# CatchMan1/AI-education-generative-recommendation

Measured on AMD Instinct MI355X. Metric: RQ-VAE items encoded/s + SASRec seqs scored/s @1/8 GPU; HR@10/NDCG@10 parity, higher is better.
Workload: dtype f32; 1 GPU; rq_c2: RQ-VAE get_indices, 3x256 codebooks, in 768 -> [256,128] -> e 32, data-derived codebooks, BERT-statistics item embeddings; global_batch=100000, parallelism=item-sharded x1, no collective

## Files before the change

ai-education-generative-recommendation_amd/_lib.py:

```python
import ctypes
import os

import torch

_PKG = os.path.dirname(os.path.abspath(__file__))
LIB_PATH = os.environ.get("GR_AMD_LIB") or os.path.join(_PKG, "lib", "libgr_amd.so")

GR_ACT_NONE = 0
GR_ACT_RELU = 1
GR_ACT_SIGMOID = 2
GR_ACT_TANH = 3
GR_ACT_LEAKYRELU = 4
GR_MAX_LEVELS = 8
GR_MAX_LINEAR = 8

_c_int_p = ctypes.POINTER(ctypes.c_int32)
_vp = ctypes.c_void_p
_i64 = ctypes.c_int64
_i32 = ctypes.c_int32
_sz = ctypes.c_size_t
_f32 = ctypes.c_float


class SasrecParams(ctypes.Structure):
    _fields_ = [("d", _i32), ("n_blocks", _i32), ("n_heads", _i32), ("mlp", _i32),
                ("max_len", _i32), ("eps", _f32), ("item_rows", _i64),
                ("item_emb", _vp), ("pos_emb", _vp),
                ("attn_ln_w", _vp), ("attn_ln_b", _vp), ("in_proj_w", _vp), ("in_proj_b", _vp),
                ("out_proj_w", _vp), ("out_proj_b", _vp), ("ffn_ln_w", _vp), ("ffn_ln_b", _vp),
                ("ffn1_w", _vp), ("ffn1_b", _vp), ("ffn2_w", _vp), ("ffn2_b", _vp),
                ("last_ln_w", _vp), ("last_ln_b", _vp)]


class SasrecTrainBufs(ctypes.Structure):
    _fields_ = [(f, _vp) for f in ("xin", "hs", "qkv", "prob", "os", "x1", "fs", "zs", "us", "xl", "g_vec")]


SIGNATURES = {
    "gr_version": (ctypes.c_char_p, []),
    "gr_last_error": (ctypes.c_char_p, []),
    "gr_set_option": (ctypes.c_int, [ctypes.c_char_p, _i64]),
    "gr_get_option": (_i64, [ctypes.c_char_p]),
    "gr_linear_f32": (ctypes.c_int, [_vp, _i64, _i32, _vp, _i32, _vp, _vp, _i64, _i32, _vp, _i64, _vp]),
    "gr_rq_codebook_norms_f32": (ctypes.c_int, [_vp, _i32, _i32, _vp, _vp]),
    "gr_rq_quantize_f32": (ctypes.c_int, [_vp, _i64, _i32, _i32, _vp, _vp, _vp, _vp, _vp, _vp, _vp]),
    "gr_rq_encode_workspace_bytes": (_sz, [_i64, _i32, _vp, _i32, _vp]),
    "gr_rq_encode_f32": (ctypes.c_int, [_vp, _i64, _i32, _vp, _vp, _vp, _i32, _vp, _vp, _vp, _vp,
                                        _vp, _vp, _vp, _sz, _vp]),
    "gr_rq_encoder_pack_floats": (_sz, [_i32, _vp]),
    "gr_rq_encoder_pack_f32": (ctypes.c_int, [_i32, _vp, _vp, _vp, _vp]),
    "gr_rq_encode_packed_f32": (ctypes.c_int, [_vp, _i64, _i32, _vp, _vp, _vp, _vp, _i32, _vp, _vp, _vp,
                                               _vp, _vp, _vp, _vp, _sz, _vp]),
    "gr_rq_mlp_workspace_bytes": (_sz, [_i64, _i32, _vp]),
    "gr_rq_mlp_f32": (ctypes.c_int, [_vp, _i64, _i32, _vp, _vp, _vp, _vp, _vp, _sz, _vp]),
    "gr_mlp_exact_f32": (ctypes.c_int, [_vp, _i64, _i32, _vp, _vp, _vp, _vp, _vp, _vp, _vp, _f32, _i32,
                                        _vp, _vp, _sz, _vp]),
    "gr_mlp_exact_groups_f32": (ctypes.c_int, [_vp, _i64, _i32, _vp, _vp, _vp, _vp, _vp, _vp, _vp, _f32,
                                               _i32, _vp, _i64, _vp, _vp]),
    "gr_mkl_plan": (_i32, [_i64, _i32, _i32, _c_int_p, _c_int_p]),
    "gr_rq_encode_sk_workspace_bytes": (_sz, [_i64, _i32, _i32, _vp]),
    "gr_rq_encode_sk_f32": (ctypes.c_int, [_vp, _i64, _i32, _i32, _vp, _vp, _vp, _i32, _vp, _i64,
                                           _vp, _vp, _sz, _vp]),
    "gr_mlp_train_fwd_f32": (ctypes.c_int, [_vp, _i64, _i32, _vp, _vp, _vp, _f32, _vp, _vp, _vp, _vp]),
    "gr_mlp_train_bwd_layer_f32": (ctypes.c_int, [_vp, _i64, _i32, _vp, _i32, _vp, _i32, _f32, _vp, _i32,
                                                  _vp, _vp, _vp, _vp]),
    "gr_rq_quantize_sk_train_f32": (ctypes.c_int, [_vp, _i64, _i32, _i32, _vp, _vp, _vp, _i32, _vp, _i64,
                                                   _vp, _vp, _vp, _vp, _sz, _vp]),
    "gr_rq_quantize_sk_train_bwd_f32": (ctypes.c_int, [_vp, _i64, _i32, _i32, _vp, _vp, _vp, _vp, _vp, _f32,
                                                       _vp, _vp, _vp]),
    "gr_sasrec_workspace_bytes": (_sz, [ctypes.POINTER(SasrecParams), _i64, _i32]),
    "gr_sasrec_forward_f32": (ctypes.c_int, [ctypes.POINTER(SasrecParams), _vp, _i64, _i32, _vp,
                                             _i32, _vp, _sz, _vp, _vp]),
    "gr_sasrec_predict_f32": (ctypes.c_int, [ctypes.POINTER(SasrecParams), _vp, _i64, _i32, _vp,
                                             _vp, _sz, _vp, _vp]),
    "gr_sasrec_predict_ld_f32": (ctypes.c_int, [ctypes.POINTER(SasrecParams), _vp, _i64, _i32, _vp,
                                                _i64, _vp, _sz, _vp, _vp]),
    "gr_sasrec_rank_workspace_bytes": (_sz, [ctypes.POINTER(SasrecParams), _i64, _i32]),
    "gr_sasrec_rank_f32": (ctypes.c_int, [ctypes.POINTER(SasrecParams), _vp, _i64, _i32, _vp, _i32, _vp, _vp,
                                          _sz, _vp, _sz, _vp, _vp]),
    "gr_sasrec_train_vec_width": (_i32, [ctypes.POINTER(SasrecParams), _i32]),
    "gr_sasrec_train_fwd_f32": (ctypes.c_int, [ctypes.POINTER(SasrecParams), _vp, _i64, _i32, _f32,
                                               ctypes.c_uint64, _vp, ctypes.POINTER(SasrecTrainBufs), _vp,
                                               _vp, _vp]),
    "gr_sasrec_train_bwd_f32": (ctypes.c_int, [ctypes.POINTER(SasrecParams), _vp, _i64, _i32, _f32,
                                               ctypes.c_uint64, _vp, ctypes.POINTER(SasrecTrainBufs), _vp,
                                               _vp, _vp]),
    "gr_sasrec_train_tiled_workspace_bytes": (_sz, [ctypes.POINTER(SasrecParams), _i64, _i32]),
    "gr_sasrec_train_tiled_parts": (_i32, [ctypes.POINTER(SasrecParams), _i64, _i32]),
    "gr_sasrec_train_tiled_fwd_f32": (ctypes.c_int, [ctypes.POINTER(SasrecParams), _vp, _i64, _i32, _f32,
                                                     ctypes.c_uint64, _vp, ctypes.POINTER(SasrecTrainBufs), _vp,
                                                     _vp, _vp, _sz, _vp]),
    "gr_sasrec_train_tiled_bwd_f32": (ctypes.c_int, [ctypes.POINTER(SasrecParams), _vp, _i64, _i32, _f32,
                                                     ctypes.c_uint64, _vp, ctypes.POINTER(SasrecTrainBufs), _vp,
                                                     _vp, _vp, _sz, _vp]),
    "gr_score_f32": (ctypes.c_int, [_vp, _i64, _i32, _vp, _i64, _vp, _i64, _vp]),
    "gr_sampled_bce_fwd_f32": (ctypes.c_int, [_vp, _i64, _i32, _i32, _vp, _i64, _vp, _vp, _i32, _f32,
                                              _vp, _vp, _vp, _vp, _vp]),
    "gr_neg_samples": (ctypes.c_int, [_vp, _i64, _i32, _i64, _i32, ctypes.c_uint64, _vp, _vp, _vp]),
    "gr_neg_samples_dseed": (ctypes.c_int, [_vp, _i64, _i32, _i64, _i32, ctypes.c_uint64, _vp, _vp, _vp, _vp]),
    "gr_sampled_bce_bwd_f32": (ctypes.c_int, [_vp, _i64, _i32, _i32, _vp, _i64, _vp, _vp, _i32, _vp,
                                              _vp, _vp, _vp, _vp]),
    "gr_rank_f32": (ctypes.c_int, [_vp, _i64, _i64, _i64, _vp, _i32, _vp, _vp]),
    "gr_count_gt_f32": (ctypes.c_int, [_vp, _i64, _i64, _i64, _vp, _vp, _vp]),
    "gr_topk_workspace_bytes": (_sz, [_i64, _i64, _i32]),
    "gr_topk_f32": (ctypes.c_int, [_vp, _i64, _i64, _i64, _i32, _i64, _vp, _vp, _vp, _vp, _vp, _sz, _vp]),
    "gr_score_pairs_f32": (ctypes.c_int, [_vp, _i64, _i32, _vp, _i64, _vp, _i32, _vp, _vp, _vp]),
    "gr_score_count_gt_f32": (ctypes.c_int, [_vp, _i64, _i32, _vp, _i64, _vp, _i32, _vp, _vp]),
    "gr_score_count_workspace_bytes": (_sz, [_i64]),
    "gr_score_count_gt_ws_f32": (ctypes.c_int, [_vp, _i64, _i32, _vp, _i64, _vp, _i32, _vp, _vp, _sz, _vp]),
    "gr_merge_topk_f32": (ctypes.c_int, [_vp, _i64, _vp, _i64, _i64, _i32, _i32, _vp, _vp, _vp]),
    "gr_merge_topk_packed": (ctypes.c_int, [_vp, _i32, _i64, _i32, _i32, _vp, _vp, _vp]),
    "gr_score_topk_workspace_bytes": (_sz, [_i64, _i32, _i64, _i32]),
    "gr_score_topk_f32": (ctypes.c_int, [_vp, _i64, _i32, _vp, _i64, _i64, _i32, _i32, _vp, _vp, _vp,
                                         _vp, _vp, _sz, _vp]),
}

_lib = None


def lib():
    global _lib
    if _lib is None:
        if not os.path.exists(LIB_PATH):
            raise RuntimeError(f"gr_amd: {LIB_PATH} is missing - run __graft_entry__.build() "
                               "(there is no CPU fallback)")
        handle = ctypes.CDLL(LIB_PATH)
        for name, (res, args) in SIGNATURES.items():
            fn = getattr(handle, name)
            fn.restype = res
            fn.argtypes = args
        _lib = handle
    return _lib


def check(rc, what):
    if rc != 0:
        msg = lib().gr_last_error().decode(errors="replace")
        raise RuntimeError(f"{what} failed (code {rc}): {msg}")


def require_gpu(*tensors):
    for t in tensors:
# ... 69 lines not shown
```

ai-education-generative-recommendation_amd/csrc/abi.cpp:

```cpp
#include <atomic>
#include <cstring>
#include <string>

#include "gr_common.h"

namespace gr {
static thread_local std::string g_last_error;
void set_error(const std::string& msg) { g_last_error = msg; }
void clear_error() { g_last_error.clear(); }

struct Opt {
  const char* name;
  std::atomic<int64_t>* v;
  int64_t lo, hi;
};
static std::atomic<int64_t> g_rq_fused{1};
static std::atomic<int64_t> g_sas_fused{2};
static std::atomic<int64_t> g_sas_rowtile{1};
static std::atomic<int64_t> g_lin_wres{1};
static std::atomic<int64_t> g_emb_proj{1};
static std::atomic<int64_t> g_topk_half{2};
static std::atomic<int64_t> g_attn_k16{1};

static const Opt kOpts[] = {
    {"rq_fused", &g_rq_fused, 0, 1},   {"sas_fused", &g_sas_fused, 0, 3}, {"sas_rowtile", &g_sas_rowtile, 0, 1},
    {"lin_wres", &g_lin_wres, 0, 1},   {"emb_proj", &g_emb_proj, 0, 1},   {"topk_half", &g_topk_half, 0, 2},
    {"attn_k16", &g_attn_k16, 0, 1},
};

static const Opt* find_opt(const char* name) {
  for (const Opt& o : kOpts)
    if (!strcmp(name, o.name)) return &o;
  return nullptr;
}

int64_t option(const char* name) {
  const Opt* o = find_opt(name);
  return o ? o->v->load() : -1;
}
}

extern "C" int gr_set_option(const char* name, int64_t value) {
  gr::clear_error();
  if (!name) return gr::fail(GR_ERR_ARG, "gr_set_option: null name");
  const gr::Opt* o = gr::find_opt(name);
  if (!o || value < o->lo || value > o->hi)
    return gr::fail(GR_ERR_ARG, std::string("gr_set_option: unknown option or value: ") + name);
  o->v->store(value);
  return GR_OK;
}

extern "C" int64_t gr_get_option(const char* name) { return name ? gr::option(name) : -1; }

extern "C" const char* gr_version(void) { return "gr_amd 0.1.0 gfx950"; }
extern "C" const char* gr_last_error(void) { return gr::g_last_error.c_str(); }
```

ai-education-generative-recommendation_amd/csrc/rq.hip:

```cpp
#include "gr_common.h"
#include "rq_quant.h"

#ifndef GR_QDIAG
#define GR_QDIAG 0
#endif

#ifndef GR_QRES
#define GR_QRES 1
#endif

namespace gr {

struct RQLevels {
  const float* cb[GR_MAX_LEVELS];
  int K[GR_MAX_LEVELS];
};

constexpr int RQ_W = 8;
constexpr int RQ_SPLIT_MAX = 3;
constexpr size_t RQ_PART_BYTES = 2 * RQ_SPLIT_MAX * 4 * 32 * 3 * sizeof(float);

template <int EP>
struct RQMaxT { static constexpr int value = EP >= 64 ? 2 : 4; };

template <int EP, int NT, bool FULL>
__device__ __forceinline__ void stage_rows(const float* __restrict__ cb, int e, int c0, int cnt, float* cbs,
                                           int tid) {
  constexpr int HQ = EP / 8;
  if (FULL) {
    for (int f = tid; f < cnt * (EP / 4); f += NT) {
      const int c = f / (EP / 4), u = f % (EP / 4), j = u >> 1, e2 = 2 * (u & 1);
      const f32x4 v = *reinterpret_cast<const f32x4*>(cb + (int64_t)(c0 + c) * EP + 4 * u);
      *reinterpret_cast<f32x2*>(cbs + cb_off<EP>(c, j) + e2) = f32x2{v[0], v[2]};
      *reinterpret_cast<f32x2*>(cbs + cb_off<EP>(c, HQ + j) + e2) = f32x2{v[1], v[3]};
    }
  } else {
    for (int f = tid; f < cnt * EP; f += NT) {
      const int c = f / EP, k = f % EP;
      cbs[feat_off<EP>(c, k)] = k < e ? cb[(int64_t)(c0 + c) * e + k] : 0.f;
    }
  }
}

template <int EP, int NT, bool FULL>
__device__ __forceinline__ void stage_norms(int e, int cnt, const float* cbs, float* cns, int tid) {
  constexpr int HQ = EP / 8;
  for (int c = tid; c < ((cnt + 31) & ~31); c += NT) {
    float s = __builtin_inff();
    if (c < cnt) {
      if (FULL) {
        float v[EP];
#pragma unroll
        for (int q = 0; q < 2 * HQ; ++q) {
          const f32x4 t = *reinterpret_cast<const f32x4*>(cbs + cb_off<EP>(c, q));
#pragma unroll
          for (int i = 0; i < 4; ++i) v[8 * (q % HQ) + 2 * i + q / HQ] = t[i];
        }
        s = GR_QDIAG == 3 ? 0.f : aten_rowsq([&](int f) { return v[f]; }, EP);
      } else {
        s = aten_rowsq([&](int f) { return cbs[feat_off<EP>(c, f)]; }, e);
      }
    }
    cns[c] = s;
  }
}

template <int EP, int NT, bool FULL>
__device__ __forceinline__ void stage_codes(const float* __restrict__ cb, int e, int c0, int cnt,
                                            float* cbs, float* cns, int tid) {
  stage_rows<EP, NT, FULL>(cb, e, c0, cnt, cbs, tid);
  __syncthreads();
  stage_norms<EP, NT, FULL>(e, cnt, cbs, cns, tid);
  __syncthreads();
}

template <int EP, bool SECOND, bool FULL>
__global__ __launch_bounds__(RQ_W * 64) void rq_quantize_kernel(
    const float* __restrict__ z, int64_t n, int e_in, int L, RQLevels lv, int kch, int64_t* __restrict__ idx_out,
    float* __restrict__ best_out, float* __restrict__ gap_out, int tiles, int split_ok, int resident) {
#pragma clang fp contract(off)
  const int e = FULL ? EP : e_in;
  static_assert(EP % 8 == 0 && EP <= 64, "e");
// ... 115 lines not shown
#pragma unroll
            for (int v = 0; v < 16; ++v) {
              const int cd = c0 + ct * 32 + (v & 3) + 8 * (v >> 2) + 4 * h;
              const float dd = fmaf(-2.f, acc[v], rn[i] + cnv[v]);
              if (GR_QDIAG == 1) {
                best[i] = fminf(best[i], acc[v]);
                continue;
              }
              const bool lt = dd < best[i];
              if (SECOND) second[i] = lt ? best[i] : fminf(second[i], dd);
              bi[i] = lt ? cd : bi[i];
              best[i] = lt ? dd : best[i];
            }
          }
        }
      }
    }
#pragma unroll
    for (int i = 0; i < RQ_MAXT; ++i) {
      if (i < my) {
        const float ob = __shfl_xor(best[i], 32), os = __shfl_xor(second[i], 32);
        const int oi = __shfl_xor(bi[i], 32);
        merge_min<SECOND>(best[i], second[i], bi[i], ob, os, oi);
      }
    }
    if (split_plan) {
      float* pl = part + (l & 1) * (RQ_SPLIT_MAX * 4 * 32 * 3);
#pragma unroll
      for (int i = 0; i < RQ_MAXT; ++i)
        if (i < my && is_split(i) && h == 0) {
          float* ep = pl + (((wk + i * WS - base) * 4 + simd) * 32 + r) * 3;
          ep[0] = best[i];
          ep[1] = second[i];
          ep[2] = __int_as_float(bi[i]);
        }
      __syncthreads();
#pragma unroll
      for (int i = 0; i < RQ_MAXT; ++i)
        if (i < my && is_split(i)) {
          const float* ep = pl + ((wk + i * WS - base) * 4 * 32 + r) * 3;
          float bb = ep[0], ss = ep[1];
          int ii = __float_as_int(ep[2]);
#pragma unroll
          for (int q = 1; q < 4; ++q)
            merge_min<SECOND>(bb, ss, ii, ep[q * 96], ep[q * 96 + 1], __float_as_int(ep[q * 96 + 2]));
          best[i] = bb;
          second[i] = ss;
          bi[i] = ii;
        }
    }
#pragma unroll
    for (int i = 0; i < RQ_MAXT; ++i) {
      if (i < my) {
        int b = bi[i];
        if (b >= K) b = 0;
        const int64_t item = (int64_t)tile_of(i) * 32 + r;
        if (h == 0 && item < n && (!is_split(i) || simd == 0)) {
          idx_out[item * L + l] = (int64_t)b;
          if (best_out) best_out[item * L + l] = best[i];
          if (gap_out) gap_out[item * L + l] = second[i] - best[i];
        }
        f32x4 cw[HQ];
        if (b >= c_last) {
#pragma unroll
          for (int j = 0; j < HQ; ++j)
            cw[j] = *reinterpret_cast<const f32x4*>(cbi + cb_off<EP>(b - c_last, HQ * h + j));
        } else {
#pragma unroll
          for (int j = 0; j < HQ; ++j)
#pragma unroll
            for (int s = 0; s < 4; ++s) {
              const int f = 8 * j + 2 * s + h;
              cw[j][s] = f < e ? cb[(int64_t)b * e + f] : 0.f;
            }
        }
#pragma unroll
        for (int j = 0; j < HQ; ++j)
#pragma unroll
          for (int s = 0; s < 4; ++s) {
            const float xq = res[i][j][s] + (cw[j][s] - res[i][j][s]);
            res[i][j][s] = res[i][j][s] - xq;
          }
      }
    }
  }
}

__global__ __launch_bounds__(256) void rq_code_norms_kernel(const float* __restrict__ cb, int K,
                                                            int e, float* __restrict__ cn) {
  const int c = blockIdx.x * 256 + threadIdx.x;
  if (c >= K) return;
  const float* row = cb + (int64_t)c * e;
  cn[c] = aten_rowsq([&](int f) { return row[f]; }, e);
}

static int cu_count() {
  static int cus = 0;
  if (!cus) {
    int dev = 0;
    if (hipGetDevice(&dev) != hipSuccess) dev = 0;
    if (hipDeviceGetAttribute(&cus, hipDeviceAttributeMultiprocessorCount, dev) != hipSuccess || cus < 1)
      cus = 256;
  }
  return cus;
}

static int launch_norms(const float* cb, int K, int e, float* cn, hipStream_t st) {
  hipLaunchKernelGGL(rq_code_norms_kernel, dim3((K + 255) / 256), dim3(256), 0, st, cb, K, e, cn);
  return check_launch("gr_rq_codebook_norms_f32");
}

template <int EP>
static int launch_quantize_e(const float* z, int64_t n, int e, int L, const RQLevels& lv, int64_t* idx,
                             float* best, float* gap, hipStream_t st) {
  int kmax = 0;
  for (int l = 0; l < L; ++l) kmax = lv.K[l] > kmax ? lv.K[l] : kmax;
  const int kch_max = 1024 * 32 / EP;
  int kch = ((kmax < kch_max ? kmax : kch_max) + 31) & ~31;
  const int64_t tiles = (n + 31) / 32;
  int ktot = 0;
  for (int l = 0; l < L; ++l) ktot += (lv.K[l] + 31) & ~31;
  const bool res = GR_QRES && tiles <= (int64_t)cu_count() &&
                   (size_t)ktot * EP * 4 + (size_t)ktot * 4 + RQ_PART_BYTES <= 160 * 1024;
  if (res) kch = ktot;
  const size_t lds = (size_t)kch * EP * 4 + (size_t)kch * 4 + RQ_PART_BYTES;
  int64_t grid = (int64_t)cu_count();
  const int64_t min_grid = (tiles + RQ_W * RQMaxT<EP>::value - 1) / (RQ_W * RQMaxT<EP>::value);
  if (grid < min_grid) grid = min_grid;
  if (grid > tiles) grid = tiles;
  if (grid > 0x7fffffffLL || tiles > 0x7fffffffLL) return fail(GR_ERR_UNSUPPORTED, "rq quantize: n too large");
  const bool full = e == EP;
  auto k = (best || gap) ? (full ? rq_quantize_kernel<EP, true, true> : rq_quantize_kernel<EP, true, false>)
                         : (full ? rq_quantize_kernel<EP, false, true> : rq_quantize_kernel<EP, false, false>);
  if (lds > 64 * 1024 &&
      hipFuncSetAttribute(reinterpret_cast<const void*>(k), hipFuncAttributeMaxDynamicSharedMemorySize,
                          (int)lds) != hipSuccess)
    return fail(GR_ERR_HIP, "rq quantize: cannot raise the LDS limit");
  hipLaunchKernelGGL(k, dim3((unsigned)grid), dim3(RQ_W * 64), lds, st, z, n, e, L, lv, kch, idx,
                     best, gap, (int)tiles, 1, res ? 1 : 0);
  return check_launch("gr_rq_quantize_f32");
}

static int launch_quantize(const float* z, int64_t n, int e, int L, const RQLevels& lv,
                           int64_t* idx, float* best, float* gap, hipStream_t st) {
  if (n == 0) return GR_OK;
  if (e <= 16) return launch_quantize_e<16>(z, n, e, L, lv, idx, best, gap, st);
  if (e <= 32) return launch_quantize_e<32>(z, n, e, L, lv, idx, best, gap, st);
  if (e <= 64) return launch_quantize_e<64>(z, n, e, L, lv, idx, best, gap, st);
  return fail(GR_ERR_UNSUPPORTED, "gr_rq_quantize_f32: e_dim must be <= 64");
}

static int check_levels(int32_t e, int32_t L, const int32_t* K, const float* const* cbs) {
  if (e < 1 || e > 4096) return fail(GR_ERR_UNSUPPORTED, "rq: 1 <= e_dim <= 4096");
  if (L < 1 || L > GR_MAX_LEVELS) return fail(GR_ERR_UNSUPPORTED, "rq: 1 <= L <= 8 levels");
  if (!K || !cbs) return fail(GR_ERR_ARG, "rq: null K / codebooks");
  for (int l = 0; l < L; ++l) {
    if (K[l] < 1) return fail(GR_ERR_ARG, "rq: codebook size must be >= 1");
    if (!cbs[l] || ((e == 16 || e == 32 || e == 64) && !aligned16(cbs[l]))) return fail(GR_ERR_ARG, "rq: codebooks must be 16-byte aligned");
  }
  return GR_OK;
}

static bool quant_chain(int64_t M, int e, int L, const int32_t* K) {
  if (e > 64) return false;
  for (int l = 0; l < L; ++l) {
    const MklPlan p = mkl_plan(M, e, K[l]);
    if (p.kind != MKL_CHAIN || p.kb < e) return false;
  }
  return true;
}

static bool mlp_chain(int64_t M, int32_t n_linear, const int32_t* dims) {
  for (int i = 0; i < n_linear; ++i) {
    const MklPlan p = mkl_plan(M, dims[i], dims[i + 1]);
    if (p.kind != MKL_CHAIN || p.kb % 2 != 0 || dims[i] % 4 != 0) return false;
  }
  return true;
}

}

extern "C" int32_t gr_mkl_plan(int64_t M, int32_t K, int32_t N, int32_t* kind, int32_t* kb) {
  const gr::MklPlan p = gr::mkl_plan(M, K, N);
  if (kind) *kind = p.kind;
  if (kb) *kb = p.kb;
  return gr::mkl_plan_pinned(M, K, N) ? 1 : 0;
}

extern "C" int gr_rq_codebook_norms_f32(const float* codebook, int32_t K, int32_t e, float* cn_out,
                                        void* stream) {
  gr::clear_error();
  if (!codebook || !cn_out || K < 1 || e < 1) return gr::fail(GR_ERR_ARG, "gr_rq_codebook_norms_f32: bad args");
  return gr::launch_norms(codebook, K, e, cn_out, reinterpret_cast<hipStream_t>(stream));
}

extern "C" int gr_rq_quantize_f32(const float* z, int64_t n, int32_t e, int32_t L, const int32_t* K,
                                  const float* const* codebooks, const float* const* code_norms,
                                  int64_t* idx_out, float* best_out, float* gap_out,
                                  void* stream) {
  using namespace gr;
  clear_error();
  (void)code_norms;
  int rc = check_levels(e, L, K, codebooks);
  if (rc) return rc;
  if (n < 0) return fail(GR_ERR_ARG, "gr_rq_quantize_f32: n < 0");
  if (n == 0) return GR_OK;
  if (!z || !idx_out || ((e == 16 || e == 32 || e == 64) && !aligned16(z))) return fail(GR_ERR_ARG, "gr_rq_quantize_f32: bad pointer");
  if (!quant_chain(n, e, L, K)) {
    const int32_t dims[1] = {e};
    return gr_rq_rows_launch(z, n, n, nullptr, 0, 0, dims, nullptr, nullptr, nullptr, nullptr, nullptr, nullptr,
                             0.f, GR_ACT_NONE, L, K, codebooks, nullptr, idx_out, best_out, gap_out,
                             reinterpret_cast<hipStream_t>(stream));
  }
  RQLevels lv{};
  for (int l = 0; l < L; ++l) {
    lv.cb[l] = codebooks[l];
    lv.K[l] = K[l];
  }
  return launch_quantize(z, n, e, L, lv, idx_out, best_out, gap_out, reinterpret_cast<hipStream_t>(stream));
}

static size_t act_bytes(int64_t n, int32_t n_linear, const int32_t* dims) {
  int widest = 0;
  for (int i = 1; i <= n_linear; ++i) widest = dims[i] > widest ? dims[i] : widest;
  return gr::align_up((size_t)n * widest * 4, 256);
}

static size_t mlp_ws_bytes(int64_t n, int32_t n_linear, const int32_t* dims) {
  return 2 * act_bytes(n, n_linear, dims) + gr::align_up(gr_rq_fused_pack_floats(n_linear, dims) * 4, 256) + 256;
}

static int mlp_exact(const float* x, int64_t n, int32_t n_linear, const int32_t* dims, const float* const* weights,
                     const float* const* biases, const float* const* bn_mean, const float* const* bn_var,
                     const float* const* bn_w, const float* const* bn_b, float bn_eps, int32_t act, float* z_out,
                     void* workspace, hipStream_t st, const float* packed = nullptr) {
  using namespace gr;
  if (!mlp_chain(n, n_linear, dims))
    return gr_rq_rows_launch(x, n, n, nullptr, 0, n_linear, dims, weights, biases, bn_mean, bn_var, bn_w, bn_b,
                             bn_eps, act, 0, nullptr, nullptr, z_out, nullptr, nullptr, nullptr, st);
  char* ws = reinterpret_cast<char*>(align_up(reinterpret_cast<uintptr_t>(workspace), 256));
  const size_t ab = act_bytes(n, n_linear, dims);
  float* buf[2] = {reinterpret_cast<float*>(ws), reinterpret_cast<float*>(ws + ab)};
  if (!bn_mean && act == GR_ACT_RELU && option("rq_fused") == 1) {
    const int rc = gr_rq_encoder_fused_launch(x, n, n_linear, dims, weights, biases, z_out,
                                              packed ? const_cast<float*>(packed) : reinterpret_cast<float*>(ws + 2 * ab),
                                              st, packed != nullptr, buf[0]);
    if (rc != GR_ERR_UNSUPPORTED) return rc;
    clear_error();
  }
  const float* cur = x;
  for (int i = 0; i < n_linear; ++i) {
    const bool last = i == n_linear - 1;
    float* out = last ? z_out : buf[i & 1];
    const bool bn = bn_mean && !last;
    const int rc = gr_linear_exact_launch(cur, n, dims[i], weights[i], dims[i + 1], biases ? biases[i] : nullptr,
                                          bn ? bn_mean[i] : nullptr, bn ? bn_var[i] : nullptr,
                                          bn && bn_w ? bn_w[i] : nullptr, bn && bn_b ? bn_b[i] : nullptr, bn_eps,
                                          last ? GR_ACT_NONE : act, out, st);
    if (rc) return rc;
    cur = out;
  }
  return GR_OK;
}

extern "C" size_t gr_rq_encode_workspace_bytes(int64_t n, int32_t n_linear, const int32_t* dims,
                                               int32_t L, const int32_t* K) {
  if (n < 0 || n_linear < 1 || !dims || L < 1 || !K) return 0;
  return mlp_ws_bytes(n, n_linear, dims) + gr::align_up((size_t)n * dims[n_linear] * 4, 256);
}

// ... 132 lines not shown
```

ai-education-generative-recommendation_amd/csrc/rq_quant.h:

```cpp
#pragma once
#include "gr_common.h"

namespace gr {

template <int EP>
__device__ __forceinline__ int cb_off(int c, int q) {
  constexpr int S = EP / 4;
  constexpr int M = S >= 8 ? 7 : S - 1;
  return c * EP + 4 * (q ^ (c & M));
}

template <int EP>
__device__ __forceinline__ int feat_off(int c, int f) {
  return cb_off<EP>(c, (f & 1) * (EP / 8) + (f >> 3)) + ((f >> 1) & 3);
}

template <int EP>
__device__ __forceinline__ float rn_exact(const f32x4 (&rr)[EP / 8], int e, int h) {
#pragma clang fp contract(off)
  constexpr int HQ = EP / 8;
  const int nv = e >> 3, full = (nv >> 2) << 2, tail = e & 7;
  float A[4], T[4];
#pragma unroll
  for (int s = 0; s < 4; ++s) {
    float a0 = 0.f, a1 = 0.f, a2 = 0.f, a3 = 0.f;
    T[s] = 0.f;
#pragma unroll
    for (int v = 0; v < HQ; ++v) {
      const float x = rr[v][s];
      const float q = x * x;
      if (v < nv) {
        const int a = v < full ? (v & 3) : 0;
        if (a == 0) a0 = a0 + q;
        else if (a == 1) a1 = a1 + q;
        else if (a == 2) a2 = a2 + q;
        else a3 = a3 + q;
      } else if (v == nv) {
        T[s] = q;
      }
    }
    A[s] = ((a0 + a1) + a2) + a3;
  }
  float PA[4], PT[4];
#pragma unroll
  for (int s = 0; s < 4; ++s) {
    PA[s] = __shfl_xor(A[s], 32);
    PT[s] = __shfl_xor(T[s], 32);
  }
  if (e < 8) {
    float a0 = 0.f, a1 = 0.f, a2 = 0.f, a3 = 0.f;
#pragma unroll
    for (int i = 0; i < 7; ++i)
      if (i < e) {
        const float q = ((i & 1) == h) ? T[i >> 1] : PT[i >> 1];
        const int k = i < ((e >> 2) << 2) ? (i & 3) : 0;
        if (k == 0) a0 = a0 + q;
        else if (k == 1) a1 = a1 + q;
        else if (k == 2) a2 = a2 + q;
        else a3 = a3 + q;
      }
    return ((a0 + a1) + a2) + a3;
  }
  float f = 0.f;
#pragma unroll
  for (int jj = 0; jj < 7; ++jj)
    if (jj < tail) f = f + (((jj & 1) == h) ? T[jj >> 1] : PT[jj >> 1]);
#pragma unroll
  for (int jj = 0; jj < 8; ++jj) f = f + (((jj & 1) == h) ? A[jj >> 1] : PA[jj >> 1]);
  return f;
}

template <bool SECOND>
__device__ __forceinline__ void merge_min(float& best, float& second, int& bi, float ob, float os, int oi) {
  const bool take = (ob < best) | ((ob == best) & (oi < bi));
  if (SECOND) second = take ? fminf(os, best) : fminf(second, ob);
  best = take ? ob : best;
  bi = take ? oi : bi;
}

}
```

include/gr_amd.h:

```cpp
#ifndef GR_AMD_H
#define GR_AMD_H

#include <stddef.h>
#include <stdint.h>

#ifdef __cplusplus
extern "C" {
#endif

#define GR_OK 0
#define GR_ERR_ARG (-1)
#define GR_ERR_UNSUPPORTED (-2)
#define GR_ERR_HIP (-3)
#define GR_ERR_WORKSPACE (-4)

#define GR_MAX_LEVELS 8
#define GR_MAX_LINEAR 8

#define GR_ACT_NONE 0
#define GR_ACT_RELU 1
#define GR_ACT_SIGMOID 2
#define GR_ACT_TANH 3
#define GR_ACT_LEAKYRELU 4

const char* gr_version(void);
const char* gr_last_error(void);
int gr_set_option(const char* name, int64_t value);
int64_t gr_get_option(const char* name);

int gr_linear_f32(const float* x, int64_t m, int32_t k, const float* w, int32_t n,
                  const float* bias, const float* residual, int64_t ldr, int32_t act,
                  float* y, int64_t ldy, void* stream);

int gr_rq_codebook_norms_f32(const float* codebook, int32_t K, int32_t e, float* cn_out, void* stream);

int gr_rq_quantize_f32(const float* z, int64_t n, int32_t e, int32_t L, const int32_t* K,
                       const float* const* codebooks, const float* const* code_norms,
                       int64_t* idx_out, float* best_out, float* gap_out, void* stream);

size_t gr_rq_encode_workspace_bytes(int64_t n, int32_t n_linear, const int32_t* dims,
                                    int32_t L, const int32_t* K);

int gr_rq_encode_f32(const float* x, int64_t n, int32_t n_linear, const int32_t* dims,
                     const float* const* weights, const float* const* biases, int32_t L,
                     const int32_t* K, const float* const* codebooks, int64_t* idx_out,
                     float* best_out, float* gap_out, float* z_out, void* workspace,
                     size_t workspace_bytes, void* stream);

size_t gr_rq_encoder_pack_floats(int32_t n_linear, const int32_t* dims);
int gr_rq_encoder_pack_f32(int32_t n_linear, const int32_t* dims, const float* const* weights,
                           float* packed, void* stream);
int gr_rq_encode_packed_f32(const float* x, int64_t n, int32_t n_linear, const int32_t* dims,
                            const float* const* weights, const float* const* biases,
                            const float* packed, int32_t L, const int32_t* K,
                            const float* const* codebooks, int64_t* idx_out, float* best_out,
                            float* gap_out, float* z_out, void* workspace, size_t workspace_bytes,
                            void* stream);

size_t gr_rq_mlp_workspace_bytes(int64_t n, int32_t n_linear, const int32_t* dims);
int gr_rq_mlp_f32(const float* x, int64_t n, int32_t n_linear, const int32_t* dims,
                  const float* const* weights, const float* const* biases, float* z_out,
                  void* workspace, size_t workspace_bytes, void* stream);

int gr_mlp_exact_f32(const float* x, int64_t n, int32_t n_linear, const int32_t* dims,
                     const float* const* weights, const float* const* biases,
                     const float* const* bn_mean, const float* const* bn_var,
                     const float* const* bn_w, const float* const* bn_b, float bn_eps,
                     int32_t act, float* z_out, void* workspace, size_t workspace_bytes,
                     void* stream);

int gr_mlp_exact_groups_f32(const float* x, int64_t n, int32_t n_linear, const int32_t* dims,
                            const float* const* weights, const float* const* biases,
                            const float* const* bn_mean, const float* const* bn_var,
                            const float* const* bn_w, const float* const* bn_b, float bn_eps,
                            int32_t act, const int64_t* group_ptr, int64_t n_groups, float* z_out,
                            void* stream);

int32_t gr_mkl_plan(int64_t M, int32_t K, int32_t N, int32_t* kind, int32_t* kb);

int gr_mlp_train_fwd_f32(const float* x, int64_t M, int32_t n_linear, const int32_t* dims,
                         const float* const* weights, const float* const* biases, float p_drop,
                         const uint64_t* seed_dev, float* xd0, float* const* outs, void* stream);

int gr_mlp_train_bwd_layer_f32(const float* xd_in, int64_t M, int32_t K, const float* weight, int32_t N,
                               const float* dz, int32_t dx_mode, float p_drop, const uint64_t* seed_dev,
                               int32_t site, float* dweight, float* dbias, float* dx_out, void* stream);

size_t gr_rq_encode_sk_workspace_bytes(int64_t n, int32_t e, int32_t L, const int32_t* K);
int gr_rq_encode_sk_f32(const float* z, int64_t n, int32_t e, int32_t L, const int32_t* K,
                        const float* const* codebooks, const double* sk_eps, int32_t sk_iters,
                        const int64_t* group_ptr, int64_t n_groups, int64_t* idx_out,
                        void* workspace, size_t workspace_bytes, void* stream);

int gr_rq_quantize_sk_train_f32(const float* z, int64_t n, int32_t e, int32_t L, const int32_t* K,
                                const float* const* codebooks, const double* sk_eps, int32_t sk_iters,
                                const int64_t* group_ptr, int64_t n_groups, int64_t* idx_out,
                                float* xq_out, float* sq_out, void* workspace, size_t workspace_bytes,
                                void* stream);

int gr_rq_quantize_sk_train_bwd_f32(const float* z, int64_t n, int32_t e, int32_t L, const int32_t* K,
                                    const float* const* codebooks, const int64_t* idx, const float* g_xq,
                                    const float* g_rq, float beta, float* dz_out,
                                    float* const* dcodebooks_out, void* stream);

typedef struct gr_sasrec_params {
  int32_t d;
  int32_t n_blocks;
  int32_t n_heads;
  int32_t mlp;
  int32_t max_len;
  float eps;
  int64_t item_rows;
  const float* item_emb;
  const float* pos_emb;
  const float* const* attn_ln_w;
  const float* const* attn_ln_b;
  const float* const* in_proj_w;
  const float* const* in_proj_b;
  const float* const* out_proj_w;
  const float* const* out_proj_b;
  const float* const* ffn_ln_w;
  const float* const* ffn_ln_b;
  const float* const* ffn1_w;
  const float* const* ffn1_b;
  const float* const* ffn2_w;
  const float* const* ffn2_b;
  const float* last_ln_w;
  const float* last_ln_b;
} gr_sasrec_params;

size_t gr_sasrec_workspace_bytes(const gr_sasrec_params* p, int64_t B, int32_t n);

int gr_sasrec_forward_f32(const gr_sasrec_params* p, const int64_t* seqs, int64_t B, int32_t n,
                          float* out, int32_t last_only, void* workspace, size_t workspace_bytes,
                          int32_t* err_flag, void* stream);

int gr_sasrec_predict_f32(const gr_sasrec_params* p, const int64_t* seqs, int64_t B, int32_t n,
                          float* logits, void* workspace, size_t workspace_bytes,
                          int32_t* err_flag, void* stream);

int gr_sasrec_predict_ld_f32(const gr_sasrec_params* p, const int64_t* seqs, int64_t B, int32_t n,
                             float* logits, int64_t ld, void* workspace, size_t workspace_bytes,
                             int32_t* err_flag, void* stream);

size_t gr_sasrec_rank_workspace_bytes(const gr_sasrec_params* p, int64_t B, int32_t n);
int gr_sasrec_rank_f32(const gr_sasrec_params* p, const int64_t* seqs, int64_t B, int32_t n,
                       const int64_t* targets, int32_t mask_col0, int64_t* ranks_out, void* workspace,
                       size_t workspace_bytes, void* count_ws, size_t count_ws_bytes, int32_t* err_flag,
                       void* stream);

typedef struct gr_sasrec_train_bufs {
  float* xin;
  float* hs;
  float* qkv;
  float* prob;
  float* os;
  float* x1;
  float* fs;
  float* zs;
  float* us;
  float* xl;
// ... 88 lines not shown
```

Baseline: 230.4 million items/s.

## Add MFMA bf16-split filter kernel for RQ nearest-code search with exact f32 rescoring

Adds a new quantize path for e=32. It computes approximate code distances with bf16 hi/lo split MFMA tiles, derives a rigorous error bound from the residual and codebook norms, and rescores in exact f32 only the candidates within that bound. It replaces the scalar f32 distance evaluation over all 256 codes per level with matrix-core work plus a small candidate walk. It is on by default through a new rq_filter option. It adds LDS staging of bf16 and f32 codebook images and divergent candidate loops, and parity rests on the bound being correct.

```diff
diff --git a/ai-education-generative-recommendation_amd/_lib.py b/ai-education-generative-recommendation_amd/_lib.py
--- a/ai-education-generative-recommendation_amd/_lib.py
+++ b/ai-education-generative-recommendation_amd/_lib.py
@@ -58,6 +58,9 @@
     "gr_mlp_exact_groups_f32": (ctypes.c_int, [_vp, _i64, _i32, _vp, _vp, _vp, _vp, _vp, _vp, _vp, _f32,
                                                _i32, _vp, _i64, _vp, _vp]),
     "gr_mkl_plan": (_i32, [_i64, _i32, _i32, _c_int_p, _c_int_p]),
+    "gr_rq_filter_bound_f32": (_f32, [_f32, _f32]),
+    "gr_rq_filter_launches": (_i64, []),
+    "gr_rq_filter_diag_counts": (None, [_vp]),
     "gr_rq_encode_sk_workspace_bytes": (_sz, [_i64, _i32, _i32, _vp]),
     "gr_rq_encode_sk_f32": (ctypes.c_int, [_vp, _i64, _i32, _i32, _vp, _vp, _vp, _i32, _vp, _i64,
                                            _vp, _vp, _sz, _vp]),
diff --git a/ai-education-generative-recommendation_amd/csrc/abi.cpp b/ai-education-generative-recommendation_amd/csrc/abi.cpp
--- a/ai-education-generative-recommendation_amd/csrc/abi.cpp
+++ b/ai-education-generative-recommendation_amd/csrc/abi.cpp
@@ -21,11 +21,12 @@
 static std::atomic<int64_t> g_emb_proj{1};
 static std::atomic<int64_t> g_topk_half{2};
 static std::atomic<int64_t> g_attn_k16{1};
+static std::atomic<int64_t> g_rq_filter{1};
 
 static const Opt kOpts[] = {
     {"rq_fused", &g_rq_fused, 0, 1},   {"sas_fused", &g_sas_fused, 0, 3}, {"sas_rowtile", &g_sas_rowtile, 0, 1},
     {"lin_wres", &g_lin_wres, 0, 1},   {"emb_proj", &g_emb_proj, 0, 1},   {"topk_half", &g_topk_half, 0, 2},
-    {"attn_k16", &g_attn_k16, 0, 1},
+    {"attn_k16", &g_attn_k16, 0, 1},   {"rq_filter", &g_rq_filter, 0, 1},
 };
 
 static const Opt* find_opt(const char* name) {
diff --git a/ai-education-generative-recommendation_amd/csrc/rq.hip b/ai-education-generative-recommendation_amd/csrc/rq.hip
--- a/ai-education-generative-recommendation_amd/csrc/rq.hip
+++ b/ai-education-generative-recommendation_amd/csrc/rq.hip
@@ -1,3 +1,5 @@
+#include <atomic>
+
 #include "gr_common.h"
 #include "rq_quant.h"
 
@@ -279,6 +281,350 @@
             res[i][j][s] = res[i][j][s] - xq;
           }
       }
+    }
+  }
+}
+
+#ifndef GR_FDIAG
+#define GR_FDIAG 0
+#endif
+#ifndef GR_FSB
+#define GR_FSB 1
+#endif
+#ifndef GR_FLIVE
+#define GR_FLIVE 1
+#endif
+#ifndef GR_FMAXT
+#define GR_FMAXT 2
+#endif
+
+typedef __bf16 bf16x8 __attribute__((ext_vector_type(8)));
+
+constexpr int RQF_KMAX = 1024;
+constexpr int RQF_F32_KMAX = 512;
+
+__device__ __forceinline__ void split_bf16(float x, __bf16& hi, __bf16& lo) {
+#pragma clang fp contract(off)
+  hi = (__bf16)x;
+  lo = (__bf16)(x - (float)hi);
+}
+
+__device__ __forceinline__ f32x16 filter_tile(const bf16x8 (&ah)[2], const bf16x8 (&al)[2], const bf16x8 (&bh)[2],
+                                              const bf16x8 (&bl)[2], f32x16 acc) {
+#pragma unroll
+  for (int t = 0; t < 2; ++t) acc = __builtin_amdgcn_mfma_f32_32x32x16_bf16(ah[t], bh[t], acc, 0, 0, 0);
+#pragma unroll
+  for (int t = 0; t < 2; ++t) acc = __builtin_amdgcn_mfma_f32_32x32x16_bf16(ah[t], bl[t], acc, 0, 0, 0);
+#pragma unroll
+  for (int t = 0; t < 2; ++t) acc = __builtin_amdgcn_mfma_f32_32x32x16_bf16(al[t], bh[t], acc, 0, 0, 0);
+  return acc;
+}
+
+template <bool LIVE>
+__global__ __launch_bounds__(RQ_W * 64) void rq_filter_kernel(
+    const float* __restrict__ z, int64_t n, int L, RQLevels lv, int kch, int f32_lds,
+    int64_t* __restrict__ idx_out, int tiles, uint32_t* __restrict__ cand_out) {
+#pragma clang fp contract(off)
+  constexpr int EP = 32, HQ = 4, W = RQ_W, NT = W * 64, MAXT = GR_FMAXT;
+  if (LIVE) f32_lds = 1;
+  extern __shared__ __attribute__((aligned(16))) float sm[];
+  float* bimg = sm;
+  float* cns = bimg + kch * EP;
+  float* wmax = cns + kch;
+  float* fimg = wmax + 16;
+  const int tid = threadIdx.x, lane = tid & 63, w = tid >> 6, r = lane & 31, h = lane >> 5;
+  const int t_begin = (int)((int64_t)blockIdx.x * tiles / gridDim.x);
+  const int t_end = (int)((int64_t)(blockIdx.x + 1) * tiles / gridDim.x);
+  const int my = (t_end - t_begin - w + W - 1) / W;
+
+  f32x4 res[MAXT][HQ];
+#pragma unroll
+  for (int i = 0; i < MAXT; ++i) {
+    const int64_t item = (int64_t)(t_begin + w + i * W) * 32 + r;
+    const bool ok = i < my && item < n;
+    const int64_t ic = ok ? item : 0;
+#pragma unroll
+    for (int j = 0; j < HQ; ++j) {
+      const f32x4 lo = *reinterpret_cast<const f32x4*>(z + ic * EP + 8 * j);
+      const f32x4 hi = *reinterpret_cast<const f32x4*>(z + ic * EP + 8 * j + 4);
+      const f32x4 v = h ? f32x4{lo[1], lo[3], hi[1], hi[3]} : f32x4{lo[0], lo[2], hi[0], hi[2]};
+      res[i][j] = ok ? v : f32x4{0.f, 0.f, 0.f, 0.f};
+    }
+  }
+
+  for (int l = 0; l < L; ++l) {
+    const int K = lv.K[l];
+    const float* __restrict__ cb = lv.cb[l];
+    const int ct_n = (K + 31) >> 5;
+    __syncthreads();
+    for (int f = tid; f < 2 * K; f += NT) {
+      const int c = f >> 1, t = f & 1;
+      float x[16];
+#pragma unroll
+      for (int q = 0; q < 4; ++q) {
+        const f32x4 v = *reinterpret_cast<const f32x4*>(cb + (int64_t)c * EP + 16 * t + 4 * q);
+#pragma unroll
+        for (int i = 0; i < 4; ++i) x[4 * q + i] = v[i];
+      }
+#pragma unroll
+      for (int hh = 0; hh < 2; ++hh) {
+        bf16x8 vh, vl;
+#pragma unroll
+        for (int i = 0; i < 8; ++i) {
+          __bf16 a, b;
+          split_bf16(x[(i < 4 ? 2 * i : 8 + 2 * (i - 4)) + hh], a, b);
+          vh[i] = a;
+          vl[i] = b;
+        }
+        *reinterpret_cast<bf16x8*>(bimg + cb_off<EP>(c, 2 * hh + t)) = vh;
+        *reinterpret_cast<bf16x8*>(bimg + cb_off<EP>(c, 4 + 2 * hh + t)) = vl;
+      }
+    }
+    if (f32_lds) stage_rows<EP, NT, true>(cb, EP, 0, K, fimg, tid);
+    float cmax = 0.f;
+    for (int c = tid; c < (LIVE ? 256 : ct_n * 32); c += NT) {
+      float s = __builtin_inff();
+      if (c < K) {
+        const float* row = cb + (int64_t)c * EP;
+        s = aten_rowsq([&](int f) { return row[f]; }, EP);
+        cmax = fmaxf(cmax, s);
+      }
+      cns[c] = s;
+    }
+    cmax = xmax<32>(xmax<16>(xmax<8>(xmax<4>(xmax<2>(xmax<1>(cmax))))));
+    if (lane == 0) wmax[w] = cmax;
+    __syncthreads();
+#pragma unroll
+    for (int i = 0; i < W; ++i) cmax = fmaxf(cmax, wmax[i]);
+
+    float rn[MAXT], m[MAXT];
+#pragma unroll
+    for (int i = 0; i < MAXT; ++i) {
+      if (!LIVE) rn[i] = rn_exact<EP>(res[i], EP, h);
+      m[i] = __builtin_inff();
+    }
+    auto split_res = [&](int i, bf16x8 (&bh)[2], bf16x8 (&bl)[2]) {
+#pragma unroll
+      for (int t = 0; t < 2; ++t)
+#pragma unroll
+        for (int q = 0; q < 8; ++q) {
+          __bf16 a, b;
+          split_bf16(-2.f * res[i][2 * t + (q >> 2)][q & 3], a, b);
+          bh[t][q] = a;
+          bl[t][q] = b;
+        }
+    };
+    auto load_codes = [&](int ct, bf16x8 (&ah)[2], bf16x8 (&al)[2], f32x16& cnv) {
+      const int code = min(ct * 32 + r, K - 1);
+#pragma unroll
+      for (int t = 0; t < 2; ++t) {
+        ah[t] = *reinterpret_cast<const bf16x8*>(bimg + cb_off<EP>(code, 2 * h + t));
+        al[t] = *reinterpret_cast<const bf16x8*>(bimg + cb_off<EP>(code, 4 + 2 * h + t));
+      }
+#pragma unroll
+      for (int g4 = 0; g4 < 4; ++g4) {
+        const f32x4 q = *reinterpret_cast<const f32x4*>(cns + ct * 32 + 8 * g4 + 4 * h);
+#pragma unroll
+        for (int i = 0; i < 4; ++i) cnv[4 * g4 + i] = q[i];
+      }
+    };
+    float thr[MAXT], best[MAXT];
+    int bi[MAXT];
+    bool allm[MAXT];
+    uint32_t ncand[MAXT];
+#pragma unroll
+    for (int i = 0; i < MAXT; ++i) {
+      best[i] = __builtin_inff();
+      bi[i] = 0x7fffffff;
+      ncand[i] = 0;
+    }
+    auto set_thr = [&](int i) {
+      m[i] = fminf(m[i], __shfl_xor(m[i], 32));
+      thr[i] = m[i] + 2.f * rq_filter_bound(rn[i], cmax);
+      allm[i] = !(fabsf(thr[i]) < __builtin_inff());
+      if (GR_FDIAG == 2) bi[i] = __float_as_int(thr[i]) & 0xff;
+    };
+    auto min16 = [](float t, const f32x16& a) {
+#pragma unroll
+      for (int v = 0; v < 16; v += 2) t = fminf(fminf(t, a[v]), a[v + 1]);
+      return t;
+    };
+    auto mark16 = [](uint32_t k, const f32x16& a, float th) {
+      const f32x16 d = th - a;
+#pragma unroll
+      for (int v = 0; v < 16; ++v) k = __builtin_amdgcn_alignbit(k, __float_as_uint(d[v]), 31);
+      return k;
+    };
+    auto walk = [&](int i, int g0, const uint32_t (&nm)[4]) {
+      if (GR_FDIAG == 1) {
+        bi[i] = min(bi[i], (int)((nm[0] ^ nm[1] ^ nm[2] ^ nm[3]) >> 1));
+        return;
+      }
+      uint32_t cm[4];
+#pragma unroll
+      for (int q = 0; q < 4; ++q) cm[q] = allm[i] ? 0xffffffffu : ~nm[q];
+      if (__builtin_amdgcn_ballot_w64((cm[0] | cm[1] | cm[2] | cm[3]) != 0) == 0) return;
+      float ev[16], od[16];
+#pragma unroll
+      for (int j = 0; j < HQ; ++j)
+#pragma unroll
+        for (int s = 0; s < 4; ++s) {
+          const float own = res[i][j][s], oth = __shfl_xor(own, 32);
+          ev[4 * j + s] = h ? oth : own;
+          od[4 * j + s] = h ? own : oth;
+        }
+      while (__builtin_amdgcn_ballot_w64((cm[0] | cm[1] | cm[2] | cm[3]) != 0) != 0) {
+        const int q = cm[0] ? 0 : cm[1] ? 1 : cm[2] ? 2 : 3;
+        const uint32_t wd = cm[0] ? cm[0] : cm[1] ? cm[1] : cm[2] ? cm[2] : cm[3];
+        const bool act = wd != 0;
+        const int p = 31 - __clz((int)(wd | 1u));
+        const uint32_t keep = ~(1u << p);
+#pragma unroll
+        for (int qq = 0; qq < 4; ++qq) cm[qq] = qq == q ? cm[qq] & keep : cm[qq];
+        const int v = 15 - (p & 15);
+        const int cd = (g0 + 2 * q + (p < 16 ? 1 : 0)) * 32 + (v & 3) + 8 * (v >> 2) + 4 * h;
+        if (act && cd < K) {
+          float cr[EP];
+          if (f32_lds) {
+#pragma unroll
+            for (int sl = 0; sl < 2 * HQ; ++sl) {
+              const f32x4 t = *reinterpret_cast<const f32x4*>(fimg + cb_off<EP>(cd, sl));
+#pragma unroll
+              for (int s = 0; s < 4; ++s) cr[8 * (sl % HQ) + 2 * s + sl / HQ] = t[s];
+            }
+          } else {
+#pragma unroll
+            for (int sl = 0; sl < EP / 4; ++sl) {
+              const f32x4 t = *reinterpret_cast<const f32x4*>(cb + (int64_t)cd * EP + 4 * sl);
+#pragma unroll
+              for (int s = 0; s < 4; ++s) cr[4 * sl + s] = t[s];
+            }
+          }
+          float chain = 0.f;
+#pragma unroll
+          for (int k = 0; k < EP; ++k) chain = fmaf(cr[k], (k & 1) ? od[k >> 1] : ev[k >> 1], chain);
+          const float dd = fmaf(-2.f, chain, rn[i] + cns[cd]);
+          const bool lt = dd < best[i];
+          bi[i] = lt ? cd : bi[i];
+          best[i] = lt ? dd : best[i];
+          ++ncand[i];
+        }
+      }
+    };
+    auto finish = [&](int i) {
+      float sec = 0.f;
+      merge_min<false>(best[i], sec, bi[i], __shfl_xor(best[i], 32), 0.f, __shfl_xor(bi[i], 32));
+      int b = bi[i];
+      if (b >= K || b < 0) b = 0;
+      const int64_t item = (int64_t)(t_begin + w + i * W) * 32 + r;
+      if (h == 0 && item < n) idx_out[item * L + l] = (int64_t)b;
+      if (GR_FDIAG == 3) {
+        const uint32_t tot = ncand[i] + __shfl_xor(ncand[i], 32);
+        if (h == 0 && item < n && cand_out) cand_out[item * L + l] = tot;
+      }
+      f32x4 cw[HQ];
+      if (f32_lds) {
+#pragma unroll
+        for (int j = 0; j < HQ; ++j) cw[j] = *reinterpret_cast<const f32x4*>(fimg + cb_off<EP>(b, HQ * h + j));
+      } else {
+#pragma unroll
+        for (int j = 0; j < HQ; ++j) {
+          const f32x4 lo = *reinterpret_cast<const f32x4*>(cb + (int64_t)b * EP + 8 * j);
+          const f32x4 hi = *reinterpret_cast<const f32x4*>(cb + (int64_t)b * EP + 8 * j + 4);
+          cw[j] = h ? f32x4{lo[1], lo[3], hi[1], hi[3]} : f32x4{lo[0], lo[2], hi[0], hi[2]};
+        }
+      }
+#pragma unroll
+      for (int j = 0; j < HQ; ++j)
+#pragma unroll
+        for (int s = 0; s < 4; ++s) {
+          const float xq = res[i][j][s] + (cw[j][s] - res[i][j][s]);
+          res[i][j][s] = res[i][j][s] - xq;
+        }
+    };
+    if constexpr (LIVE) {
+#pragma unroll
+      for (int i = 0; i < MAXT; ++i) {
+        if (i < my && GR_FDIAG == 4) {
+          rn[i] = 0.f;
+          finish(i);
+        } else if (i < my) {
+          f32x16 acc[8];
+          float t = __builtin_inff();
+          bf16x8 bh[2], bl[2];
+          split_res(i, bh, bl);
+          rn[i] = rn_exact<EP>(res[i], EP, h);
+#pragma unroll
+          for (int u = 0; u < 8; ++u)
+          {
+            bf16x8 ah[2], al[2];
+            f32x16 cnv;
+            load_codes(u, ah, al, cnv);
+            acc[u] = filter_tile(ah, al, bh, bl, cnv);
+#if GR_FSB
+            t = min16(t, acc[u]);
+            __builtin_amdgcn_sched_barrier(0);
+#endif
+          }
+#if !GR_FSB
+#pragma unroll
+          for (int u = 0; u < 8; ++u) t = min16(t, acc[u]);
+#endif
+          m[i] = t;
+          set_thr(i);
+          if (GR_FDIAG == 2) {
+            finish(i);
+            continue;
+          }
+          uint32_t nm[4];
+#pragma unroll
+          for (int u = 0; u < 8; ++u) {
+            nm[u >> 1] = mark16((u & 1) ? nm[u >> 1] : 0u, acc[u], thr[i]);
+            __builtin_amdgcn_sched_barrier(0);
+          }
+          walk(i, 0, nm);
+          finish(i);
+        }
+      }
+    } else {
+      bf16x8 bh[MAXT][2], bl[MAXT][2];
+#pragma unroll
+      for (int i = 0; i < MAXT; ++i) split_res(i, bh[i], bl[i]);
+#pragma unroll 1
+      for (int ct = 0; ct < (GR_FDIAG == 4 ? 0 : ct_n); ++ct) {
+        bf16x8 ah[2], al[2];
+        f32x16 cnv;
+        load_codes(ct, ah, al, cnv);
+#pragma unroll
+        for (int i = 0; i < MAXT; ++i)
+          if (i < my) m[i] = min16(m[i], filter_tile(ah, al, bh[i], bl[i], cnv));
+      }
+#pragma unroll
+      for (int i = 0; i < MAXT; ++i) set_thr(i);
+      for (int g0 = 0; g0 < (GR_FDIAG == 2 || GR_FDIAG == 4 ? 0 : ct_n); g0 += 8) {
+        uint32_t nmk[MAXT][4];
+#pragma unroll
+        for (int u = 0; u < 8; ++u) {
+          if (g0 + u < ct_n) {
+            bf16x8 ah[2], al[2];
+            f32x16 cnv;
+            load_codes(g0 + u, ah, al, cnv);
+#pragma unroll
+            for (int i = 0; i < MAXT; ++i)
+              if (i < my)
+                nmk[i][u >> 1] = mark16((u & 1) ? nmk[i][u >> 1] : 0u, filter_tile(ah, al, bh[i], bl[i], cnv), thr[i]);
+          } else {
+#pragma unroll
+            for (int i = 0; i < MAXT; ++i) nmk[i][u >> 1] = (((u & 1) ? nmk[i][u >> 1] : 0u) << 16) | 0xffffu;
+          }
+        }
+#pragma unroll
+        for (int i = 0; i < MAXT; ++i)
+          if (i < my) walk(i, g0, nmk[i]);
+      }
+#pragma unroll
+      for (int i = 0; i < MAXT; ++i)
+        if (i < my) finish(i);
     }
   }
 }
@@ -338,9 +684,44 @@
   return check_launch("gr_rq_quantize_f32");
 }
 
+static std::atomic<int64_t> g_filter_launches{0};
+static std::atomic<uint32_t*> g_filter_counts{nullptr};
+
+static bool filter_ok(int e, int L, const RQLevels& lv, const float* best, const float* gap) {
+  if (e != 32 || best || gap || option("rq_filter") != 1) return false;
+  for (int l = 0; l < L; ++l)
+    if (lv.K[l] > RQF_KMAX) return false;
+  return true;
+}
+
+static int launch_filter(const float* z, int64_t n, int L, const RQLevels& lv, int64_t* idx, hipStream_t st) {
+  int kmax = 0;
+  for (int l = 0; l < L; ++l) kmax = lv.K[l] > kmax ? lv.K[l] : kmax;
+  const bool live = GR_FLIVE && kmax <= 256;
+  const int kch = live ? 256 : (kmax + 31) & ~31;
+  const int f32_lds = kch <= RQF_F32_KMAX;
+  const size_t lds = (size_t)kch * 32 * 4 * (f32_lds ? 2 : 1) + (size_t)kch * 4 + 16 * 4;
+  const int64_t tiles = (n + 31) / 32;
+  int64_t grid = (int64_t)cu_count();
+  const int64_t min_grid = (tiles + RQ_W * GR_FMAXT - 1) / (RQ_W * GR_FMAXT);
+  if (grid < min_grid) grid = min_grid;
+  if (grid > tiles) grid = tiles;
+  if (grid > 0x7fffffffLL || tiles > 0x7fffffffLL) return fail(GR_ERR_UNSUPPORTED, "rq quantize: n too large");
+  auto k = live ? rq_filter_kernel<true> : rq_filter_kernel<false>;
+  if (lds > 64 * 1024 &&
+      hipFuncSetAttribute(reinterpret_cast<const void*>(k),
+                          hipFuncAttributeMaxDynamicSharedMemorySize, (int)lds) != hipSuccess)
+    return fail(GR_ERR_HIP, "rq quantize: cannot raise the LDS limit");
+  hipLaunchKernelGGL(k, dim3((unsigned)grid), dim3(RQ_W * 64), lds, st, z, n, L, lv, kch, f32_lds,
+                     idx, (int)tiles, g_filter_counts.load());
+  g_filter_launches.fetch_add(1);
+  return check_launch("gr_rq_quantize_f32");
+}
+
 static int launch_quantize(const float* z, int64_t n, int e, int L, const RQLevels& lv,
                            int64_t* idx, float* best, float* gap, hipStream_t st) {
   if (n == 0) return GR_OK;
+  if (filter_ok(e, L, lv, best, gap)) return launch_filter(z, n, L, lv, idx, st);
   if (e <= 16) return launch_quantize_e<16>(z, n, e, L, lv, idx, best, gap, st);
   if (e <= 32) return launch_quantize_e<32>(z, n, e, L, lv, idx, best, gap, st);
   if (e <= 64) return launch_quantize_e<64>(z, n, e, L, lv, idx, best, gap, st);
@@ -383,6 +764,12 @@
   if (kb) *kb = p.kb;
   return gr::mkl_plan_pinned(M, K, N) ? 1 : 0;
 }
+
+extern "C" float gr_rq_filter_bound_f32(float rn, float cmax2) { return gr::rq_filter_bound(rn, cmax2); }
+
+extern "C" int64_t gr_rq_filter_launches(void) { return gr::g_filter_launches.load(); }
+
+extern "C" void gr_rq_filter_diag_counts(uint32_t* counts) { gr::g_filter_counts.store(counts); }
 
 extern "C" int gr_rq_codebook_norms_f32(const float* codebook, int32_t K, int32_t e, float* cn_out,
                                         void* stream) {
diff --git a/ai-education-generative-recommendation_amd/csrc/rq_quant.h b/ai-education-generative-recommendation_amd/csrc/rq_quant.h
--- a/ai-education-generative-recommendation_amd/csrc/rq_quant.h
+++ b/ai-education-generative-recommendation_amd/csrc/rq_quant.h
@@ -78,4 +78,10 @@
   bi = take ? oi : bi;
 }
 
+__host__ __device__ inline float rq_filter_bound(float rn, float cmax2) {
+#pragma clang fp contract(off)
+  const float R = __builtin_sqrtf(rn), C = __builtin_sqrtf(cmax2);
+  return (0x1p-13f * (R * C) + 0x1p-15f * (rn + cmax2)) + 0x1p-116f * ((R + C) + 1.f);
 }
+
+}
diff --git a/include/gr_amd.h b/include/gr_amd.h
--- a/include/gr_amd.h
+++ b/include/gr_amd.h
@@ -77,6 +77,10 @@
                             void* stream);
 
 int32_t gr_mkl_plan(int64_t M, int32_t K, int32_t N, int32_t* kind, int32_t* kb);
+
+float gr_rq_filter_bound_f32(float rn, float cmax2);
+int64_t gr_rq_filter_launches(void);
+void gr_rq_filter_diag_counts(uint32_t* counts);
 
 int gr_mlp_train_fwd_f32(const float* x, int64_t M, int32_t n_linear, const int32_t* dims,
                          const float* const* weights, const float* const* biases, float p_drop,
```

Result: faster. 243.9 million items/s (median of 6 runs) (+5.9%).
